# lyuchenyang/Macaw-LLM

Measured on NVIDIA H100. Metric: multimodal prefill tokens/sec (img+audio+text->LLaMA), higher is better.
Workload: dtype fp16

## Files before the change

### macaw-llm_b200/csrc/gemm_wgmma.cu

```cuda
#include "common.cuh"
#include "ptx.cuh"
#include "../../include/macaw_b200.h"
#include <stdlib.h>

namespace mm {

struct GemmKParams {
  int M, N, K, batch, batch2;
  int m_tiles, n_tiles, num_k;
  int b_shared, b2_shared;
  void* C;
  long long ldc, c_bs, c_bs2;
  int c_fp32;
  int act;
  float alpha;
  const bf16* bias;
  long long bias_bs;
  const float* row_scale;
  const bf16* residual;
  long long ldr, r_bs, r_bs2;
  int res_row_mod;
  const float* rope_cos;
  const float* rope_sin;
  int rope_T, rope_cols;
// ... 589 lines not shown
            phase ^= 1;
          }
        }
      }
    }
    return;
  }

  const int q = warp & 3;
  const float* srow = sC + (q * 32 + lane) * LDS;
  if (EWG && warp >= 8) {
    if constexpr (EWG) setmaxnreg_inc<168>();
    GemmWork wk;
    for (int it = 0; gemm_work(p, worker, n_workers, total_tiles, it, wk); ++it) {
      const TileCoord t = tile_coord(wk.tile, p, m_units);
      const float rs = epi_row_scale(p, t, t.m_blk * kBlockM + q * 32 + lane);
      mbar_wait(staging_full, it & 1);
      for (int half = 0; half < 2; ++half) gemm_epilogue<BN, EPI>(p, t, wk, srow, rs, q, lane, half, q + 4 * half, worker, n_workers);
      mbar_arrive(staging_empty);
    }
    return;
  }

  if constexpr (EWG) setmaxnreg_inc<152>();
  const int wg = warp >> 2;
  int stage = 0;
  uint32_t phase = 0;
  GemmWork wk;
  for (int it = 0; gemm_work(p, worker, n_workers, total_tiles, it, wk); ++it) {
    const TileCoord t = tile_coord(wk.tile, p, m_units);
    {
      float acc[BN / 2];
#pragma unroll
      for (int i = 0; i < BN / 2; ++i) acc[i] = 0.f;
      int prev = -1;
      for (int kb = wk.kb0; kb < wk.kb1; ++kb) {
        mbar_wait(&full_bar[stage], phase);
        const uint32_t a_addr = smem_u32(sA + stage * kABytes) + wg * 8192;
        const uint32_t b_addr = smem_u32(sB + stage * B_BYTES);
        const uint64_t a_desc = make_sdesc_sw128(a_addr, A_MN ? 8192 : 16, 1024);
        const uint64_t b_desc = make_sdesc_sw128(b_addr, B_MN ? 8192 : 16, 1024);
        wgmma_fence();
#pragma unroll
        for (int kk = 0; kk < kBlockK / 16; ++kk)
          wgmma_tile<BN, F16, A_MN ? 1 : 0, B_MN ? 1 : 0>(acc, a_desc + static_cast<uint64_t>(A_MN ? kk * 128 : kk * 2),
                                                         b_desc + static_cast<uint64_t>(B_MN ? kk * 128 : kk * 2));
        wgmma_commit();
        wgmma_wait<1>();
        if (prev >= 0) {
          __syncwarp();
          if (lane == 0) mbar_arrive(&empty_bar[prev]);
        }
        prev = stage;
        if (++stage == STAGES) {
          stage = 0;
          phase ^= 1;
        }
      }
      wgmma_wait<0>();
      fence_regs(acc);
      __syncwarp();
      if (lane == 0) mbar_arrive(&empty_bar[prev]);
      if constexpr (EWG) mbar_wait(staging_empty, (it & 1) ^ 1);
      else consumer_sync();
      const int r0 = wg * 64 + q * 16 + (lane >> 2);
      const int c0 = 2 * (lane & 3);
#pragma unroll
      for (int j = 0; j < BN / 8; ++j) {
        *reinterpret_cast<float2*>(sC + r0 * LDS + 8 * j + c0) = make_float2(acc[4 * j], acc[4 * j + 1]);
        *reinterpret_cast<float2*>(sC + (r0 + 8) * LDS + 8 * j + c0) = make_float2(acc[4 * j + 2], acc[4 * j + 3]);
      }
      if constexpr (EWG) {
        mbar_arrive(staging_full);
        continue;
      }
      consumer_sync();
    }
    const int half = warp >> 2;
    const float rs = wk.role == 1 ? 1.0f : epi_row_scale(p, t, t.m_blk * kBlockM + q * 32 + lane);
    gemm_epilogue<BN, EPI>(p, t, wk, srow, rs, q, lane, half, warp, worker, n_workers);
  }
}

typedef CUresult (*EncodeTiledFn)(CUtensorMap*, CUtensorMapDataType, cuuint32_t, void*, const cuuint64_t*,
                                  const cuuint64_t*, const cuuint32_t*, const cuuint32_t*, CUtensorMapInterleave,
                                  CUtensorMapSwizzle, CUtensorMapL2promotion, CUtensorMapFloatOOBfill);

static EncodeTiledFn get_encode_fn() {
  static EncodeTiledFn fn = nullptr;
  if (fn == nullptr) {
    void* p = nullptr;
    cudaDriverEntryPointQueryResult q;
    if (cudaGetDriverEntryPoint("cuTensorMapEncodeTiled", &p, cudaEnableDefault, &q) == cudaSuccess &&
        q == cudaDriverEntryPointSuccess)
      fn = reinterpret_cast<EncodeTiledFn>(p);
  }
  return fn;
}

int make_map(CUtensorMap* m, const void* ptr, uint64_t inner, uint64_t rows, uint64_t batch, uint64_t batch2,
             int64_t ld, int64_t bs, int64_t bs2, uint32_t box_rows) {
  EncodeTiledFn fn = get_encode_fn();
  if (fn == nullptr) {
    set_error("cuTensorMapEncodeTiled entry point unavailable (no CUDA driver?)");
    return 1;
  }
  cuuint64_t dims[4] = {inner, rows, batch, batch2};
  if (bs <= 0) bs = static_cast<int64_t>(rows) * ld;
  if (bs2 <= 0) bs2 = static_cast<int64_t>(batch) * bs;
  cuuint64_t strides[3] = {static_cast<cuuint64_t>(ld) * 2, static_cast<cuuint64_t>(bs) * 2,
                           static_cast<cuuint64_t>(bs2) * 2};
  cuuint32_t box[4] = {64, box_rows, 1, 1};
  cuuint32_t estr[4] = {1, 1, 1, 1};
  CUresult r = fn(m, CU_TENSOR_MAP_DATA_TYPE_BFLOAT16, 4, const_cast<void*>(ptr), dims, strides, box, estr,
                  CU_TENSOR_MAP_INTERLEAVE_NONE, CU_TENSOR_MAP_SWIZZLE_128B, CU_TENSOR_MAP_L2_PROMOTION_L2_256B,
                  CU_TENSOR_MAP_FLOAT_OOB_FILL_NONE);
  if (r != CUDA_SUCCESS) {
    set_error("cuTensorMapEncodeTiled failed (%d): ptr=%p dims={%llu,%llu,%llu,%llu} ld=%lld bs=%lld bs2=%lld box_rows=%u",
              static_cast<int>(r), ptr, (unsigned long long)inner, (unsigned long long)rows,
              (unsigned long long)batch, (unsigned long long)batch2, (long long)ld, (long long)bs, (long long)bs2,
              box_rows);
    return 1;
  }
  return 0;
}


static int& streamk_mode() {
  static int mode = []() { const char* e = getenv("MACAW_B200_GEMM_STREAMK"); const int v = e ? atoi(e) : 1; return v < 0 || v > 2 ? 1 : v; }();
  return mode;
}

static int& overlap_mode() {
  static int mode = []() { const char* e = getenv("MACAW_B200_GEMM_OVERLAP"); const int v = e ? atoi(e) : 1; return v < 0 || v > 1 ? 1 : v; }();
  return mode;
}

template <int BN, int EPI, bool B_MN, bool A_MN = false>
static int launch_gemm(const CUtensorMap& ta, const CUtensorMap& tb, const GemmKParams& p, bool f16, bool ewg,
                       cudaStream_t st) {
  if (ewg && p.sk_tiles != 0) {
    set_error("mm_gemm_fwd: the epilogue-warpgroup kernel takes no stream-K tail");
    return 1;
  }
  static bool attr_set[2][2][kMaxDevices] = {};
  constexpr size_t smem = gemm_smem_bytes(BN);
  auto kern = f16 ? (ewg ? gemm_bf16_kernel<BN, EPI, B_MN, A_MN, true, true> : gemm_bf16_kernel<BN, EPI, B_MN, A_MN, true, false>)
                  : (ewg ? gemm_bf16_kernel<BN, EPI, B_MN, A_MN, false, true> : gemm_bf16_kernel<BN, EPI, B_MN, A_MN, false, false>);
  if (int rc = ensure_smem_attr(kern, smem, attr_set[f16 ? 1 : 0][ewg ? 1 : 0], "mm_gemm_fwd")) return rc;
  const int total = p.batch * p.batch2 * p.m_tiles * p.n_tiles;
  const int grid = (total < num_sms() && p.sk_tiles == 0) ? total : num_sms();
  cudaError_t e = launch_kernel(kern, dim3(grid), dim3(ewg ? kGemmThreadsEwg : kGemmThreads), smem, st, 1, ta, tb, p);
  if (e != cudaSuccess) {
    set_error("mm_gemm_fwd: launch failed: %s", cudaGetErrorString(e));
    return 2;
  }
  return check_launch("mm_gemm_fwd");
}

}

using namespace mm;

static int32_t gemm_dispatch(const mm_gemm_args* a, void* stream, mm_gemm_schedule* plan) {
  MM_REQUIRE(a != nullptr, "mm_gemm_fwd: null args");
  MM_REQUIRE(a->M > 0 && a->N > 0 && a->K > 0 && a->batch > 0 && a->batch2 >= 0,
             "mm_gemm_fwd: bad shape M=%d N=%d K=%d batch=%d batch2=%d", a->M, a->N, a->K, a->batch, a->batch2);
  const int batch2 = a->batch2 > 0 ? a->batch2 : 1;
  MM_REQUIRE(a->A && a->B && a->C, "mm_gemm_fwd: null operand");
  MM_REQUIRE((reinterpret_cast<uintptr_t>(a->A) & 15) == 0 && (reinterpret_cast<uintptr_t>(a->B) & 15) == 0,
             "mm_gemm_fwd: A/B must be 16-byte aligned");
  MM_REQUIRE(a->lda % 8 == 0 && a->ldb % 8 == 0, "mm_gemm_fwd: lda/ldb must be multiples of 8 elements (lda=%lld ldb=%lld)",
             (long long)a->lda, (long long)a->ldb);
  MM_REQUIRE(a->batch == 1 || (a->a_bs % 8 == 0 && a->b_bs % 8 == 0), "mm_gemm_fwd: batch strides must be multiples of 8");
  MM_REQUIRE(batch2 == 1 || (a->a_bs2 % 8 == 0 && a->b_bs2 % 8 == 0), "mm_gemm_fwd: batch2 strides must be multiples of 8");
  MM_REQUIRE(a->epi >= MM_EPI_STD && a->epi <= MM_EPI_ROPE, "mm_gemm_fwd: bad epilogue %d", a->epi);

  GemmKParams p;
  p.M = a->M; p.N = a->N; p.K = a->K; p.batch = a->batch; p.batch2 = batch2;
  p.num_k = (a->K + kBlockK - 1) / kBlockK;
  p.m_tiles = (a->M + kBlockM - 1) / kBlockM;
  p.b_shared = (a->batch > 1 && a->b_bs == 0) ? 1 : 0;
  p.b2_shared = (batch2 > 1 && a->b_bs2 == 0) ? 1 : 0;
  p.C = a->C; p.ldc = a->ldc; p.c_bs = a->c_bs; p.c_bs2 = a->c_bs2; p.c_fp32 = a->c_fp32;
  p.act = a->act; p.alpha = a->alpha;
  p.bias = reinterpret_cast<const bf16*>(a->bias); p.bias_bs = a->bias_bs;
  p.row_scale = a->row_scale;
  p.residual = reinterpret_cast<const bf16*>(a->residual); p.ldr = a->ldr; p.r_bs = a->r_bs; p.r_bs2 = a->r_bs2;
  p.res_row_mod = a->res_row_mod;
  p.rope_cos = a->rope_cos; p.rope_sin = a->rope_sin; p.rope_T = a->rope_T; p.rope_cols = a->rope_cols;
  p.rope_pos = a->rope_pos;
  p.c_trans = a->c_trans;
  p.c_fp16 = a->c_fp16;
  p.aux_f16 = act_f16() ? 1 : 0;
  p.bias_rs = a->bias_rs; p.bias2 = reinterpret_cast<const bf16*>(a->bias2); p.bias2_rs = a->bias2_rs;
  p.sumsq_out = a->sumsq_out; p.sumsq_parts = (a->N + 31) / 32;
  p.rs_sumsq = a->rs_sumsq; p.rs_parts = a->rs_parts; p.rs_eps = a->rs_eps;
  MM_REQUIRE(a->sumsq_out == nullptr || (a->epi == MM_EPI_STD && !a->c_trans && !a->c_fp32 && a->batch == 1 && batch2 == 1 &&
                                         a->N % 32 == 0),
             "mm_gemm_fwd: sumsq_out needs the standard epilogue, 16-bit output, no batching and N %% 32 == 0");
  MM_REQUIRE(a->rs_sumsq == nullptr || (a->rs_parts > 0 && a->rs_parts % 4 == 0 && !a->c_trans && a->batch == 1 && batch2 == 1 &&
                                        (reinterpret_cast<uintptr_t>(a->rs_sumsq) & 15) == 0),
             "mm_gemm_fwd: rs_sumsq needs rs_parts %% 4 == 0, a 16-byte aligned buffer and no batching");
  MM_REQUIRE(!(a->c_fp16 && a->c_fp32), "mm_gemm_fwd: c_fp16 and c_fp32 are exclusive");
  MM_REQUIRE((a->a_fp16 != 0) == (a->b_fp16 != 0),
             "mm_gemm_fwd: A and B must share one 16-bit format (wgmma takes no mixed f16 x bf16 operands)");
  MM_REQUIRE((!a->bias_rs && !a->bias2 && !a->bias2_rs) || (a->epi == MM_EPI_STD && !a->c_trans),
             "mm_gemm_fwd: row-scaled bias terms need the standard, non-transposed epilogue");
  MM_REQUIRE(!(a->c_fp16 && a->c_fp32), "mm_gemm_fwd: c_fp16 and c_fp32 are exclusive");
  MM_REQUIRE(!a->c_trans || (a->epi == MM_EPI_STD && a->batch == 1 && batch2 == 1),
             "mm_gemm_fwd: c_trans needs the standard epilogue and no batching");

  const int esz = a->c_fp32 ? 4 : 2;
  bool vec = (reinterpret_cast<uintptr_t>(a->C) % 16 == 0) && ((a->ldc * esz) % 16 == 0) &&
             ((a->c_bs * esz) % 16 == 0) && ((a->c_bs2 * esz) % 16 == 0);
  if (a->bias) vec = vec && (reinterpret_cast<uintptr_t>(a->bias) % 16 == 0) && (a->bias_bs % 8 == 0);
  if (a->residual)
    vec = vec && (reinterpret_cast<uintptr_t>(a->residual) % 16 == 0) && (a->ldr % 8 == 0) && (a->r_bs % 8 == 0) &&
          (a->r_bs2 % 8 == 0);
  p.vec_ok = vec ? 1 : 0;

  const int sms = num_sms();
  int BN = kMaxBN;
  if (a->epi == MM_EPI_ROPE) {
    MM_REQUIRE(a->N % 128 == 0 && a->rope_cos && a->rope_sin && a->rope_T > 0 && vec && a->rope_cols % 128 == 0,
               "mm_gemm_fwd: RoPE epilogue needs N %% 128 == 0, cos/sin tables and vector-aligned C");
  } else if (a->epi == MM_EPI_SWIGLU) {
    MM_REQUIRE(a->N % 64 == 0, "mm_gemm_fwd: SwiGLU epilogue needs N %% 64 == 0");
  } else {
    const int cands[3] = {128, 64, 32};
    const long long kcost[3] = {512, 282, 192};
    long long best = -1;
    BN = 32;
    for (int i = 0; i < 3; ++i) {
      const int bn = cands[i];
      if (a->b_mn_major && bn < 64) continue;
      if (bn > 32 && a->N <= bn / 2) continue;
      const long long tiles = (long long)a->batch * batch2 * p.m_tiles * ((a->N + bn - 1) / bn);
      const long long waves = (tiles + sms - 1) / sms;
      const long long cost = waves * ((long long)p.num_k * kcost[i] + 2 * kcost[i]);
      if (best < 0 || cost < best) {
        best = cost;
        BN = bn;
      }
    }
    if (a->b_mn_major && BN < 64) BN = 64;
  }
  p.n_tiles = (a->N + BN - 1) / BN;
  static const int gm_env = []() { const char* e = getenv("MACAW_B200_GEMM_GROUPM"); return e ? atoi(e) : 0; }();
  const long long tiles = (long long)a->batch * batch2 * p.m_tiles * p.n_tiles;
  {
    const long long unit_bytes = (long long)kBlockM * a->K * 2;
    long long g = ((16LL << 20) + unit_bytes / 2) / unit_bytes;
    g = g < 2 ? 2 : (g > 32 ? 32 : g);
    p.group_m = gm_env > 0 ? gm_env : static_cast<int>(g);
  }
  p.sk_tiles = 0; p.sk_first = 0; p.sk_ws = nullptr; p.sk_flags = nullptr;
  const int sk_env = streamk_mode();
  if (sk_env != 0 && a->sk_workspace != nullptr && p.num_k >= 8 && tiles > sms &&
      static_cast<long long>(sms) * p.num_k * (sms + 1) < (1LL << 31)) {
    const int rem = static_cast<int>(tiles % sms);
    const long long need = 8192 + static_cast<long long>(sms) * kBlockM * BN * 4;
    const bool pays = sk_env == 2 || static_cast<long long>(sms - rem) * p.num_k * BN >= 3400LL * 256;
    if (rem > 0 && pays && a->sk_workspace_bytes >= need &&
        (reinterpret_cast<uintptr_t>(a->sk_workspace) & 15) == 0) {
      p.sk_tiles = rem;
      p.sk_first = static_cast<int>(tiles - rem);
      p.sk_flags = reinterpret_cast<int*>(a->sk_workspace);
      p.sk_ws = reinterpret_cast<float*>(reinterpret_cast<char*>(a->sk_workspace) + 8192);
    }
  }
  MM_REQUIRE(!a->a_mn_major || (a->b_mn_major && a->epi == MM_EPI_STD && !a->c_trans),
             "mm_gemm_fwd: MN-major A needs MN-major B and the standard epilogue");
  MM_REQUIRE(!a->b_mn_major || a->epi == MM_EPI_STD, "mm_gemm_fwd: MN-major B only with the standard epilogue");
  if (plan != nullptr) {
    plan->block_n = BN;
    plan->pairs = 0;
    plan->m_tiles = p.m_tiles;
    plan->n_tiles = p.n_tiles;
    plan->k_blocks = p.num_k;
    plan->units = tiles;
    plan->workers = sms;
    plan->grid = static_cast<int>((tiles < sms && p.sk_tiles == 0) ? tiles : sms);
    plan->waves = static_cast<int>((tiles + sms - 1) / sms);
    plan->group_m = p.group_m;
    plan->streamk_tiles = p.sk_tiles;
    plan->smem_bytes = static_cast<int32_t>(gemm_smem_bytes(BN));
    plan->vectorised_epilogue = p.vec_ok;
    return 0;
  }
  CUtensorMap ta, tb;
  if (a->a_mn_major) {
    if (make_map(&ta, a->A, a->M, a->K, a->batch, batch2, a->lda, a->a_bs, a->a_bs2, 64)) return 1;
  } else if (make_map(&ta, a->A, a->K, a->M, a->batch, batch2, a->lda, a->a_bs, a->a_bs2, kBlockM)) {
    return 1;
  }
  const uint64_t b_batch = p.b_shared ? 1 : a->batch;
  const uint64_t b_batch2 = p.b2_shared ? 1 : batch2;
  if (!a->b_mn_major) {
    if (make_map(&tb, a->B, a->K, a->N, b_batch, b_batch2, a->ldb, a->b_bs, a->b_bs2, BN)) return 1;
  } else {
    if (make_map(&tb, a->B, a->N, a->K, b_batch, b_batch2, a->ldb, a->b_bs, a->b_bs2, 64)) return 1;
  }
  cudaStream_t st = reinterpret_cast<cudaStream_t>(stream);
  const bool f16 = a->a_fp16 != 0;
  const bool ewg = overlap_mode() == 1 && p.num_k >= kEwgMinKBlocks && p.sk_tiles == 0;

#define MM_LAUNCH(BN_, EPI_, MN_) return launch_gemm<BN_, EPI_, MN_>(ta, tb, p, f16, ewg, st)
  if (a->epi == MM_EPI_ROPE) MM_LAUNCH(128, MM_EPI_ROPE, false);
  if (a->epi == MM_EPI_SWIGLU) MM_LAUNCH(128, MM_EPI_SWIGLU, false);
  if (a->a_mn_major) {
    if (BN == 128) return launch_gemm<128, MM_EPI_STD, true, true>(ta, tb, p, f16, ewg, st);
    return launch_gemm<64, MM_EPI_STD, true, true>(ta, tb, p, f16, ewg, st);
  }
  if (a->b_mn_major) {
    if (BN == 128) MM_LAUNCH(128, MM_EPI_STD, true);
    MM_LAUNCH(64, MM_EPI_STD, true);
  }
  if (BN == 128) MM_LAUNCH(128, MM_EPI_STD, false);
  if (BN == 64) MM_LAUNCH(64, MM_EPI_STD, false);
  MM_LAUNCH(32, MM_EPI_STD, false);
#undef MM_LAUNCH
}

extern "C" int32_t mm_gemm_fwd(const mm_gemm_args* a, void* stream) { return gemm_dispatch(a, stream, nullptr); }

extern "C" int32_t mm_gemm_plan(const mm_gemm_args* a, mm_gemm_schedule* plan) {
  MM_REQUIRE(plan != nullptr, "mm_gemm_plan: null plan");
  return gemm_dispatch(a, nullptr, plan);
}

extern "C" int32_t mm_gemm_streamk_mode(int32_t mode) {
  const int prev = streamk_mode();
  if (mode >= 0 && mode <= 2) streamk_mode() = mode;
  return prev;
}

extern "C" int32_t mm_gemm_overlap_mode(int32_t mode) {
  const int prev = overlap_mode();
  if (mode >= 0 && mode <= 1) overlap_mode() = mode;
  return prev;
}

extern "C" int64_t mm_gemm_streamk_workspace_bytes(void) {
  return 8192 + static_cast<int64_t>(num_sms()) * kBlockM * kMaxBN * 4;
}


namespace mm {
__global__ void splitk_reduce_kernel(const float* __restrict__ part, int splits, int M, int N,
                                     const bf16* __restrict__ bias, bf16* __restrict__ out, long long ldo, int out_fp16,
                                     int bias_f16) {
  const long long total = static_cast<long long>(M) * N;
  for (long long i = blockIdx.x * static_cast<long long>(blockDim.x) + threadIdx.x; i < total;
       i += static_cast<long long>(gridDim.x) * blockDim.x) {
    const int m = static_cast<int>(i / N), n = static_cast<int>(i % N);
    float acc = bias ? aux_ld(bias, n, bias_f16) : 0.0f;
    for (int s = 0; s < splits; ++s) acc += part[static_cast<long long>(s) * total + i];
    if (out_fp16)
      reinterpret_cast<__half*>(out)[static_cast<long long>(m) * ldo + n] = __float2half_rn(acc);
    else
      out[static_cast<long long>(m) * ldo + n] = __float2bfloat16(acc);
  }
}
}

extern "C" int32_t mm_splitk_reduce(const float* partial, int32_t splits, int32_t M, int32_t N, const void* bias,
                                    void* out, int64_t ldo, int32_t out_fp16, void* stream) {
  MM_REQUIRE(partial && out && splits > 0 && M > 0 && N > 0, "mm_splitk_reduce: bad arguments");
  const long long total = static_cast<long long>(M) * N;
  int blocks = static_cast<int>((total + 255) / 256);
  if (blocks > num_sms() * 8) blocks = num_sms() * 8;
  splitk_reduce_kernel<<<blocks, 256, 0, reinterpret_cast<cudaStream_t>(stream)>>>(
      partial, splits, M, N, reinterpret_cast<const bf16*>(bias), reinterpret_cast<bf16*>(out), ldo, out_fp16,
      act_f16() ? 1 : 0);
  return check_launch("mm_splitk_reduce");
}
```

### macaw-llm_b200/csrc/ptx.cuh

```cuda
#pragma once
#include <cuda_runtime.h>
#include <cuda_bf16.h>
#include <cuda_fp16.h>
#include <cuda.h>
#include <stdint.h>

namespace mm {

__device__ __forceinline__ uint32_t smem_u32(const void* p) {
  return static_cast<uint32_t>(__cvta_generic_to_shared(p));
}

__device__ __forceinline__ uint32_t lane_id() { return threadIdx.x & 31; }

__device__ __forceinline__ uint32_t elect_one() {
  uint32_t pred = 0;
  asm volatile(
      "{\n"
      ".reg .pred px;\n"
      "elect.sync _|px, 0xFFFFFFFF;\n"
      "selp.b32 %0, 1, 0, px;\n"
      "}\n"
      : "=r"(pred));
  return pred;
// ... 74 lines not shown
      : "memory");
}
constexpr uint64_t kEvictNormal = 0x1000000000000000ull;
constexpr uint64_t kEvictFirst = 0x12F0000000000000ull;
constexpr uint64_t kEvictLast = 0x14F0000000000000ull;

__device__ __forceinline__ uint64_t make_sdesc_sw128(uint32_t smem_addr, uint32_t lbo_bytes, uint32_t sbo_bytes) {
  uint64_t d = 0;
  d |= static_cast<uint64_t>((smem_addr & 0x3FFFF) >> 4);
  d |= static_cast<uint64_t>((lbo_bytes >> 4) & 0x3FFF) << 16;
  d |= static_cast<uint64_t>((sbo_bytes >> 4) & 0x3FFF) << 32;
  d |= static_cast<uint64_t>(1) << 62;
  return d;
}

__device__ __forceinline__ void wgmma_fence() { asm volatile("wgmma.fence.sync.aligned;" ::: "memory"); }
__device__ __forceinline__ void wgmma_commit() { asm volatile("wgmma.commit_group.sync.aligned;" ::: "memory"); }
template <int N>
__device__ __forceinline__ void wgmma_wait() {
  asm volatile("wgmma.wait_group.sync.aligned %0;" ::"n"(N) : "memory");
}
template <int N>
__device__ __forceinline__ void fence_regs(float (&d)[N]) {
#pragma unroll
  for (int i = 0; i < N; ++i) asm volatile("" : "+f"(d[i])::"memory");
}

__device__ __forceinline__ void stage_ld32(const float* s, uint32_t (&r)[32]) {
#pragma unroll
  for (int i = 0; i < 8; ++i) {
    const float4 f = reinterpret_cast<const float4*>(s)[i];
    r[4 * i] = __float_as_uint(f.x);
    r[4 * i + 1] = __float_as_uint(f.y);
    r[4 * i + 2] = __float_as_uint(f.z);
    r[4 * i + 3] = __float_as_uint(f.w);
  }
}

template <bool F16, int TA, int TB>
__device__ __forceinline__ void wgmma_ss_n32(float (&d)[16], uint64_t a, uint64_t b, uint32_t scale_d) {
  if constexpr (F16)
    asm volatile(
        "{\n.reg .pred p;\nsetp.ne.b32 p, %18, 0;\n"
        "wgmma.mma_async.sync.aligned.m64n32k16.f32.f16.f16 {%0, %1, %2, %3, %4, %5, %6, %7, %8, %9, %10, %11, %12, %13, %14, %15}, %16, %17, p, 1, 1, %19, %20;\n}\n"
        : "+f"(d[0]), "+f"(d[1]), "+f"(d[2]), "+f"(d[3]), "+f"(d[4]), "+f"(d[5]), "+f"(d[6]), "+f"(d[7]), "+f"(d[8]), "+f"(d[9]), "+f"(d[10]), "+f"(d[11]), "+f"(d[12]), "+f"(d[13]), "+f"(d[14]), "+f"(d[15])
        : "l"(a), "l"(b), "r"(scale_d), "n"(TA), "n"(TB));
  else
    asm volatile(
        "{\n.reg .pred p;\nsetp.ne.b32 p, %18, 0;\n"
        "wgmma.mma_async.sync.aligned.m64n32k16.f32.bf16.bf16 {%0, %1, %2, %3, %4, %5, %6, %7, %8, %9, %10, %11, %12, %13, %14, %15}, %16, %17, p, 1, 1, %19, %20;\n}\n"
        : "+f"(d[0]), "+f"(d[1]), "+f"(d[2]), "+f"(d[3]), "+f"(d[4]), "+f"(d[5]), "+f"(d[6]), "+f"(d[7]), "+f"(d[8]), "+f"(d[9]), "+f"(d[10]), "+f"(d[11]), "+f"(d[12]), "+f"(d[13]), "+f"(d[14]), "+f"(d[15])
        : "l"(a), "l"(b), "r"(scale_d), "n"(TA), "n"(TB));
}
template <bool F16, int TA, int TB>
__device__ __forceinline__ void wgmma_ss_n64(float (&d)[32], uint64_t a, uint64_t b, uint32_t scale_d) {
  if constexpr (F16)
    asm volatile(
        "{\n.reg .pred p;\nsetp.ne.b32 p, %34, 0;\n"
        "wgmma.mma_async.sync.aligned.m64n64k16.f32.f16.f16 {%0, %1, %2, %3, %4, %5, %6, %7, %8, %9, %10, %11, %12, %13, %14, %15, %16, %17, %18, %19, %20, %21, %22, %23, %24, %25, %26, %27, %28, %29, %30, %31}, %32, %33, p, 1, 1, %35, %36;\n}\n"
        : "+f"(d[0]), "+f"(d[1]), "+f"(d[2]), "+f"(d[3]), "+f"(d[4]), "+f"(d[5]), "+f"(d[6]), "+f"(d[7]), "+f"(d[8]), "+f"(d[9]), "+f"(d[10]), "+f"(d[11]), "+f"(d[12]), "+f"(d[13]), "+f"(d[14]), "+f"(d[15]), "+f"(d[16]), "+f"(d[17]), "+f"(d[18]), "+f"(d[19]), "+f"(d[20]), "+f"(d[21]), "+f"(d[22]), "+f"(d[23]), "+f"(d[24]), "+f"(d[25]), "+f"(d[26]), "+f"(d[27]), "+f"(d[28]), "+f"(d[29]), "+f"(d[30]), "+f"(d[31])
        : "l"(a), "l"(b), "r"(scale_d), "n"(TA), "n"(TB));
  else
    asm volatile(
        "{\n.reg .pred p;\nsetp.ne.b32 p, %34, 0;\n"
        "wgmma.mma_async.sync.aligned.m64n64k16.f32.bf16.bf16 {%0, %1, %2, %3, %4, %5, %6, %7, %8, %9, %10, %11, %12, %13, %14, %15, %16, %17, %18, %19, %20, %21, %22, %23, %24, %25, %26, %27, %28, %29, %30, %31}, %32, %33, p, 1, 1, %35, %36;\n}\n"
        : "+f"(d[0]), "+f"(d[1]), "+f"(d[2]), "+f"(d[3]), "+f"(d[4]), "+f"(d[5]), "+f"(d[6]), "+f"(d[7]), "+f"(d[8]), "+f"(d[9]), "+f"(d[10]), "+f"(d[11]), "+f"(d[12]), "+f"(d[13]), "+f"(d[14]), "+f"(d[15]), "+f"(d[16]), "+f"(d[17]), "+f"(d[18]), "+f"(d[19]), "+f"(d[20]), "+f"(d[21]), "+f"(d[22]), "+f"(d[23]), "+f"(d[24]), "+f"(d[25]), "+f"(d[26]), "+f"(d[27]), "+f"(d[28]), "+f"(d[29]), "+f"(d[30]), "+f"(d[31])
        : "l"(a), "l"(b), "r"(scale_d), "n"(TA), "n"(TB));
}
template <bool F16, int TA, int TB>
__device__ __forceinline__ void wgmma_ss_n128(float (&d)[64], uint64_t a, uint64_t b, uint32_t scale_d) {
  if constexpr (F16)
    asm volatile(
        "{\n.reg .pred p;\nsetp.ne.b32 p, %66, 0;\n"
        "wgmma.mma_async.sync.aligned.m64n128k16.f32.f16.f16 {%0, %1, %2, %3, %4, %5, %6, %7, %8, %9, %10, %11, %12, %13, %14, %15, %16, %17, %18, %19, %20, %21, %22, %23, %24, %25, %26, %27, %28, %29, %30, %31, %32, %33, %34, %35, %36, %37, %38, %39, %40, %41, %42, %43, %44, %45, %46, %47, %48, %49, %50, %51, %52, %53, %54, %55, %56, %57, %58, %59, %60, %61, %62, %63}, %64, %65, p, 1, 1, %67, %68;\n}\n"
        : "+f"(d[0]), "+f"(d[1]), "+f"(d[2]), "+f"(d[3]), "+f"(d[4]), "+f"(d[5]), "+f"(d[6]), "+f"(d[7]), "+f"(d[8]), "+f"(d[9]), "+f"(d[10]), "+f"(d[11]), "+f"(d[12]), "+f"(d[13]), "+f"(d[14]), "+f"(d[15]), "+f"(d[16]), "+f"(d[17]), "+f"(d[18]), "+f"(d[19]), "+f"(d[20]), "+f"(d[21]), "+f"(d[22]), "+f"(d[23]), "+f"(d[24]), "+f"(d[25]), "+f"(d[26]), "+f"(d[27]), "+f"(d[28]), "+f"(d[29]), "+f"(d[30]), "+f"(d[31]), "+f"(d[32]), "+f"(d[33]), "+f"(d[34]), "+f"(d[35]), "+f"(d[36]), "+f"(d[37]), "+f"(d[38]), "+f"(d[39]), "+f"(d[40]), "+f"(d[41]), "+f"(d[42]), "+f"(d[43]), "+f"(d[44]), "+f"(d[45]), "+f"(d[46]), "+f"(d[47]), "+f"(d[48]), "+f"(d[49]), "+f"(d[50]), "+f"(d[51]), "+f"(d[52]), "+f"(d[53]), "+f"(d[54]), "+f"(d[55]), "+f"(d[56]), "+f"(d[57]), "+f"(d[58]), "+f"(d[59]), "+f"(d[60]), "+f"(d[61]), "+f"(d[62]), "+f"(d[63])
        : "l"(a), "l"(b), "r"(scale_d), "n"(TA), "n"(TB));
  else
    asm volatile(
        "{\n.reg .pred p;\nsetp.ne.b32 p, %66, 0;\n"
        "wgmma.mma_async.sync.aligned.m64n128k16.f32.bf16.bf16 {%0, %1, %2, %3, %4, %5, %6, %7, %8, %9, %10, %11, %12, %13, %14, %15, %16, %17, %18, %19, %20, %21, %22, %23, %24, %25, %26, %27, %28, %29, %30, %31, %32, %33, %34, %35, %36, %37, %38, %39, %40, %41, %42, %43, %44, %45, %46, %47, %48, %49, %50, %51, %52, %53, %54, %55, %56, %57, %58, %59, %60, %61, %62, %63}, %64, %65, p, 1, 1, %67, %68;\n}\n"
        : "+f"(d[0]), "+f"(d[1]), "+f"(d[2]), "+f"(d[3]), "+f"(d[4]), "+f"(d[5]), "+f"(d[6]), "+f"(d[7]), "+f"(d[8]), "+f"(d[9]), "+f"(d[10]), "+f"(d[11]), "+f"(d[12]), "+f"(d[13]), "+f"(d[14]), "+f"(d[15]), "+f"(d[16]), "+f"(d[17]), "+f"(d[18]), "+f"(d[19]), "+f"(d[20]), "+f"(d[21]), "+f"(d[22]), "+f"(d[23]), "+f"(d[24]), "+f"(d[25]), "+f"(d[26]), "+f"(d[27]), "+f"(d[28]), "+f"(d[29]), "+f"(d[30]), "+f"(d[31]), "+f"(d[32]), "+f"(d[33]), "+f"(d[34]), "+f"(d[35]), "+f"(d[36]), "+f"(d[37]), "+f"(d[38]), "+f"(d[39]), "+f"(d[40]), "+f"(d[41]), "+f"(d[42]), "+f"(d[43]), "+f"(d[44]), "+f"(d[45]), "+f"(d[46]), "+f"(d[47]), "+f"(d[48]), "+f"(d[49]), "+f"(d[50]), "+f"(d[51]), "+f"(d[52]), "+f"(d[53]), "+f"(d[54]), "+f"(d[55]), "+f"(d[56]), "+f"(d[57]), "+f"(d[58]), "+f"(d[59]), "+f"(d[60]), "+f"(d[61]), "+f"(d[62]), "+f"(d[63])
        : "l"(a), "l"(b), "r"(scale_d), "n"(TA), "n"(TB));
}
template <bool F16, int TB>
__device__ __forceinline__ void wgmma_rs_n64(float (&d)[32], const uint32_t (&a)[4], uint64_t b, uint32_t scale_d) {
  if constexpr (F16)
    asm volatile(
        "{\n.reg .pred p;\nsetp.ne.b32 p, %37, 0;\n"
        "wgmma.mma_async.sync.aligned.m64n64k16.f32.f16.f16 {%0, %1, %2, %3, %4, %5, %6, %7, %8, %9, %10, %11, %12, %13, %14, %15, %16, %17, %18, %19, %20, %21, %22, %23, %24, %25, %26, %27, %28, %29, %30, %31}, {%32, %33, %34, %35}, %36, p, 1, 1, %38;\n}\n"
        : "+f"(d[0]), "+f"(d[1]), "+f"(d[2]), "+f"(d[3]), "+f"(d[4]), "+f"(d[5]), "+f"(d[6]), "+f"(d[7]), "+f"(d[8]), "+f"(d[9]), "+f"(d[10]), "+f"(d[11]), "+f"(d[12]), "+f"(d[13]), "+f"(d[14]), "+f"(d[15]), "+f"(d[16]), "+f"(d[17]), "+f"(d[18]), "+f"(d[19]), "+f"(d[20]), "+f"(d[21]), "+f"(d[22]), "+f"(d[23]), "+f"(d[24]), "+f"(d[25]), "+f"(d[26]), "+f"(d[27]), "+f"(d[28]), "+f"(d[29]), "+f"(d[30]), "+f"(d[31])
        : "r"(a[0]), "r"(a[1]), "r"(a[2]), "r"(a[3]), "l"(b), "r"(scale_d), "n"(TB));
  else
    asm volatile(
        "{\n.reg .pred p;\nsetp.ne.b32 p, %37, 0;\n"
        "wgmma.mma_async.sync.aligned.m64n64k16.f32.bf16.bf16 {%0, %1, %2, %3, %4, %5, %6, %7, %8, %9, %10, %11, %12, %13, %14, %15, %16, %17, %18, %19, %20, %21, %22, %23, %24, %25, %26, %27, %28, %29, %30, %31}, {%32, %33, %34, %35}, %36, p, 1, 1, %38;\n}\n"
        : "+f"(d[0]), "+f"(d[1]), "+f"(d[2]), "+f"(d[3]), "+f"(d[4]), "+f"(d[5]), "+f"(d[6]), "+f"(d[7]), "+f"(d[8]), "+f"(d[9]), "+f"(d[10]), "+f"(d[11]), "+f"(d[12]), "+f"(d[13]), "+f"(d[14]), "+f"(d[15]), "+f"(d[16]), "+f"(d[17]), "+f"(d[18]), "+f"(d[19]), "+f"(d[20]), "+f"(d[21]), "+f"(d[22]), "+f"(d[23]), "+f"(d[24]), "+f"(d[25]), "+f"(d[26]), "+f"(d[27]), "+f"(d[28]), "+f"(d[29]), "+f"(d[30]), "+f"(d[31])
        : "r"(a[0]), "r"(a[1]), "r"(a[2]), "r"(a[3]), "l"(b), "r"(scale_d), "n"(TB));
}
template <bool F16, int TB>
__device__ __forceinline__ void wgmma_rs_n128(float (&d)[64], const uint32_t (&a)[4], uint64_t b, uint32_t scale_d) {
  if constexpr (F16)
    asm volatile(
        "{\n.reg .pred p;\nsetp.ne.b32 p, %69, 0;\n"
        "wgmma.mma_async.sync.aligned.m64n128k16.f32.f16.f16 {%0, %1, %2, %3, %4, %5, %6, %7, %8, %9, %10, %11, %12, %13, %14, %15, %16, %17, %18, %19, %20, %21, %22, %23, %24, %25, %26, %27, %28, %29, %30, %31, %32, %33, %34, %35, %36, %37, %38, %39, %40, %41, %42, %43, %44, %45, %46, %47, %48, %49, %50, %51, %52, %53, %54, %55, %56, %57, %58, %59, %60, %61, %62, %63}, {%64, %65, %66, %67}, %68, p, 1, 1, %70;\n}\n"
        : "+f"(d[0]), "+f"(d[1]), "+f"(d[2]), "+f"(d[3]), "+f"(d[4]), "+f"(d[5]), "+f"(d[6]), "+f"(d[7]), "+f"(d[8]), "+f"(d[9]), "+f"(d[10]), "+f"(d[11]), "+f"(d[12]), "+f"(d[13]), "+f"(d[14]), "+f"(d[15]), "+f"(d[16]), "+f"(d[17]), "+f"(d[18]), "+f"(d[19]), "+f"(d[20]), "+f"(d[21]), "+f"(d[22]), "+f"(d[23]), "+f"(d[24]), "+f"(d[25]), "+f"(d[26]), "+f"(d[27]), "+f"(d[28]), "+f"(d[29]), "+f"(d[30]), "+f"(d[31]), "+f"(d[32]), "+f"(d[33]), "+f"(d[34]), "+f"(d[35]), "+f"(d[36]), "+f"(d[37]), "+f"(d[38]), "+f"(d[39]), "+f"(d[40]), "+f"(d[41]), "+f"(d[42]), "+f"(d[43]), "+f"(d[44]), "+f"(d[45]), "+f"(d[46]), "+f"(d[47]), "+f"(d[48]), "+f"(d[49]), "+f"(d[50]), "+f"(d[51]), "+f"(d[52]), "+f"(d[53]), "+f"(d[54]), "+f"(d[55]), "+f"(d[56]), "+f"(d[57]), "+f"(d[58]), "+f"(d[59]), "+f"(d[60]), "+f"(d[61]), "+f"(d[62]), "+f"(d[63])
        : "r"(a[0]), "r"(a[1]), "r"(a[2]), "r"(a[3]), "l"(b), "r"(scale_d), "n"(TB));
  else
    asm volatile(
        "{\n.reg .pred p;\nsetp.ne.b32 p, %69, 0;\n"
        "wgmma.mma_async.sync.aligned.m64n128k16.f32.bf16.bf16 {%0, %1, %2, %3, %4, %5, %6, %7, %8, %9, %10, %11, %12, %13, %14, %15, %16, %17, %18, %19, %20, %21, %22, %23, %24, %25, %26, %27, %28, %29, %30, %31, %32, %33, %34, %35, %36, %37, %38, %39, %40, %41, %42, %43, %44, %45, %46, %47, %48, %49, %50, %51, %52, %53, %54, %55, %56, %57, %58, %59, %60, %61, %62, %63}, {%64, %65, %66, %67}, %68, p, 1, 1, %70;\n}\n"
        : "+f"(d[0]), "+f"(d[1]), "+f"(d[2]), "+f"(d[3]), "+f"(d[4]), "+f"(d[5]), "+f"(d[6]), "+f"(d[7]), "+f"(d[8]), "+f"(d[9]), "+f"(d[10]), "+f"(d[11]), "+f"(d[12]), "+f"(d[13]), "+f"(d[14]), "+f"(d[15]), "+f"(d[16]), "+f"(d[17]), "+f"(d[18]), "+f"(d[19]), "+f"(d[20]), "+f"(d[21]), "+f"(d[22]), "+f"(d[23]), "+f"(d[24]), "+f"(d[25]), "+f"(d[26]), "+f"(d[27]), "+f"(d[28]), "+f"(d[29]), "+f"(d[30]), "+f"(d[31]), "+f"(d[32]), "+f"(d[33]), "+f"(d[34]), "+f"(d[35]), "+f"(d[36]), "+f"(d[37]), "+f"(d[38]), "+f"(d[39]), "+f"(d[40]), "+f"(d[41]), "+f"(d[42]), "+f"(d[43]), "+f"(d[44]), "+f"(d[45]), "+f"(d[46]), "+f"(d[47]), "+f"(d[48]), "+f"(d[49]), "+f"(d[50]), "+f"(d[51]), "+f"(d[52]), "+f"(d[53]), "+f"(d[54]), "+f"(d[55]), "+f"(d[56]), "+f"(d[57]), "+f"(d[58]), "+f"(d[59]), "+f"(d[60]), "+f"(d[61]), "+f"(d[62]), "+f"(d[63])
        : "r"(a[0]), "r"(a[1]), "r"(a[2]), "r"(a[3]), "l"(b), "r"(scale_d), "n"(TB));
}

__device__ __forceinline__ uint32_t pack_bf16x2(float lo, float hi) {
  __nv_bfloat162 v = __floats2bfloat162_rn(lo, hi);
  return *reinterpret_cast<uint32_t*>(&v);
}
__device__ __forceinline__ uint32_t pack_f16x2(float lo, float hi) {
  __half2 v = __floats2half2_rn(lo, hi);
  return *reinterpret_cast<uint32_t*>(&v);
}
__device__ __forceinline__ float bf16lo(uint32_t v) { return __uint_as_float(v << 16); }
__device__ __forceinline__ float bf16hi(uint32_t v) { return __uint_as_float(v & 0xFFFF0000u); }

template <bool F16>
__device__ __forceinline__ float cvt_in(uint16_t raw) {
  if constexpr (F16) return __half2float(__ushort_as_half(raw));
  return __uint_as_float(static_cast<uint32_t>(raw) << 16);
}
template <bool F16>
__device__ __forceinline__ uint16_t cvt_out(float v) {
  if constexpr (F16) return __half_as_ushort(__float2half_rn(v));
  return __bfloat16_as_ushort(__float2bfloat16(v));
}
template <bool F16>
__device__ __forceinline__ uint32_t pack2(float lo, float hi) {
  if constexpr (F16) return pack_f16x2(lo, hi);
  return pack_bf16x2(lo, hi);
}
template <bool F16>
__device__ __forceinline__ void unpack2(uint32_t v, float& lo, float& hi) {
  if constexpr (F16) {
    const float2 f = __half22float2(*reinterpret_cast<const __half2*>(&v));
    lo = f.x;
    hi = f.y;
  } else {
    lo = bf16lo(v);
    hi = bf16hi(v);
  }
}
template <bool F16>
__device__ __forceinline__ void unpack8t(const uint4& u, float (&f)[8]) {
  unpack2<F16>(u.x, f[0], f[1]);
  unpack2<F16>(u.y, f[2], f[3]);
  unpack2<F16>(u.z, f[4], f[5]);
  unpack2<F16>(u.w, f[6], f[7]);
}
template <bool F16>
__device__ __forceinline__ uint4 pack8t(const float (&f)[8]) {
  return make_uint4(pack2<F16>(f[0], f[1]), pack2<F16>(f[2], f[3]), pack2<F16>(f[4], f[5]), pack2<F16>(f[6], f[7]));
}
template <bool F16>
__device__ __forceinline__ float ldv(__nv_bfloat16 v) { return cvt_in<F16>(__bfloat16_as_ushort(v)); }
template <bool F16>
__device__ __forceinline__ __nv_bfloat16 stv(float v) { return __ushort_as_bfloat16(cvt_out<F16>(v)); }
// ... 3 lines not shown
```

Measured before the change: 33500.

## Add wide 128x256 wgmma GEMM kernel with dedicated epilogue warpgroup

Adds a persistent GEMM kernel in which each CTA computes a pair of adjacent N tiles (BN=256) using m64n256k16 wgmma, with two consumer warpgroups and a third warpgroup handling the epilogue through a staged shared-memory tile. Loading the wider B tile per A tile raises operand reuse and halves the A traffic per output. The default overlap mode becomes 2, which routes large non-batched, K-major GEMMs with an even number of N tiles to this kernel. The trade-offs are fewer pipeline stages (3), higher register pressure handled via setmaxnreg, and a serialized two-sided epilogue handoff.

```diff
diff --git a/macaw-llm_b200/csrc/gemm_wgmma.cu b/macaw-llm_b200/csrc/gemm_wgmma.cu
--- a/macaw-llm_b200/csrc/gemm_wgmma.cu
+++ b/macaw-llm_b200/csrc/gemm_wgmma.cu
@@ -695,6 +695,164 @@
   }
 }
 
+constexpr int kWideThreads = 384;
+constexpr int kWideStages = 3;
+constexpr uint32_t kWideBBytes = 2 * kMaxBN * kBlockK * 2;
+constexpr size_t kWideSmemBytes =
+    1024 + kWideStages * (kABytes + kWideBBytes) + (size_t)kBlockM * gemm_stage_ld(kMaxBN) * 4 + 256;
+static_assert(kWideSmemBytes <= 227 * 1024, "wide GEMM: ring + staging tile exceed an sm_90 block's shared memory");
+constexpr int kWideRegsConsumer = 184, kWideRegsEpilogue = 136;
+static_assert(2 * kWideRegsConsumer + kWideRegsEpilogue <= 3 * 168, "wide GEMM: register budget");
+
+__device__ __forceinline__ TileCoord pair_coord(int idx, const GemmKParams& p) {
+  const int n_pairs = p.n_tiles / 2;
+  const int in_group = p.group_m * n_pairs;
+  const int g = idx / in_group;
+  const int first_m = g * p.group_m;
+  const int gsz = min(p.m_tiles - first_m, p.group_m);
+  const int rr = idx - g * in_group;
+  TileCoord t;
+  t.b = t.b_lo = t.b_hi = 0;
+  t.m_blk = first_m + rr % gsz;
+  t.n_blk = 2 * (rr / gsz);
+  return t;
+}
+
+template <int EPI, bool F16>
+__global__ void __launch_bounds__(kWideThreads, 1)
+gemm_wide_kernel(const __grid_constant__ CUtensorMap tmA, const __grid_constant__ CUtensorMap tmB, const GemmKParams p) {
+  constexpr int BN = kMaxBN;
+  constexpr int LDS = gemm_stage_ld(BN);
+  extern __shared__ uint8_t smem_raw[];
+  uint8_t* smem = reinterpret_cast<uint8_t*>((reinterpret_cast<uintptr_t>(smem_raw) + 1023) & ~uintptr_t(1023));
+  uint8_t* sA = smem;
+  uint8_t* sB = smem + kWideStages * kABytes;
+  float* sC = reinterpret_cast<float*>(sB + kWideStages * kWideBBytes);
+  uint64_t* full_bar = reinterpret_cast<uint64_t*>(sC + kBlockM * LDS);
+  uint64_t* empty_bar = full_bar + kWideStages;
+  uint64_t* staging_full = empty_bar + kWideStages;
+  uint64_t* staging_empty = staging_full + 1;
+
+  const int warp = threadIdx.x >> 5;
+  const int lane = threadIdx.x & 31;
+  const int worker = static_cast<int>(blockIdx.x);
+  const int n_workers = static_cast<int>(gridDim.x);
+  const int total_pairs = p.m_tiles * (p.n_tiles / 2);
+
+  if (warp == 0 && elect_one()) {
+    tma_prefetch_desc(&tmA);
+    tma_prefetch_desc(&tmB);
+    for (int s = 0; s < kWideStages; ++s) {
+      mbar_init(&full_bar[s], 1);
+      mbar_init(&empty_bar[s], 8);
+    }
+    mbar_init(staging_full, 256);
+    mbar_init(staging_empty, 128);
+    fence_mbar_init();
+  }
+  __syncthreads();
+  griddep_launch();
+  griddep_wait();
+
+  const int q = warp & 3;
+  if (warp >= 8) {
+    setmaxnreg_dec<kWideRegsEpilogue>();
+    const float* srow = sC + (q * 32 + lane) * LDS;
+    GemmWork wk;
+    wk.tile = 0; wk.kb0 = 0; wk.kb1 = p.num_k; wk.role = 0; wk.c0 = 0; wk.nc = 0;
+    for (int u = worker; u < total_pairs; u += n_workers) {
+      TileCoord t = pair_coord(u, p);
+      const float rs = epi_row_scale(p, t, t.m_blk * kBlockM + q * 32 + lane);
+#pragma unroll 1
+      for (int side = 0; side < 2; ++side) {
+        mbar_wait(staging_full, side);
+        for (int half = 0; half < 2; ++half)
+          gemm_epilogue<BN, EPI>(p, t, wk, srow, rs, q, lane, half, q + 4 * half, worker, n_workers);
+        mbar_arrive(staging_empty);
+        ++t.n_blk;
+      }
+    }
+    return;
+  }
+
+  setmaxnreg_inc<kWideRegsConsumer>();
+  const int wg = warp >> 2;
+  int stage = 0;
+  uint32_t phase = 0;
+  const bool loader = threadIdx.x == 0;
+  int ld_u = worker, ld_kb = 0, ld_stage = 0;
+  uint32_t ld_phase = 0;
+  TileCoord ld_t = pair_coord(worker, p);
+  auto load_next = [&]() {
+    if (ld_u >= total_pairs) return;
+    mbar_wait(&empty_bar[ld_stage], ld_phase ^ 1);
+    mbar_arrive_expect_tx(&full_bar[ld_stage], kABytes + kWideBBytes);
+    tma_load_4d(&tmA, &full_bar[ld_stage], sA + ld_stage * kABytes, ld_kb * kBlockK, ld_t.m_blk * kBlockM, 0, 0);
+    uint8_t* b = sB + ld_stage * kWideBBytes;
+    tma_load_4d(&tmB, &full_bar[ld_stage], b, ld_kb * kBlockK, ld_t.n_blk * BN, 0, 0);
+    tma_load_4d(&tmB, &full_bar[ld_stage], b + kWideBBytes / 2, ld_kb * kBlockK, (ld_t.n_blk + 1) * BN, 0, 0);
+    if (++ld_stage == kWideStages) {
+      ld_stage = 0;
+      ld_phase ^= 1;
+    }
+    if (++ld_kb == p.num_k) {
+      ld_kb = 0;
+      ld_u += n_workers;
+      if (ld_u < total_pairs) ld_t = pair_coord(ld_u, p);
+    }
+  };
+  if (loader)
+    for (int s = 0; s < kWideStages; ++s) load_next();
+  __syncwarp();
+  for (int u = worker; u < total_pairs; u += n_workers) {
+    float acc[2 * BN / 2];
+#pragma unroll
+    for (int i = 0; i < BN; ++i) acc[i] = 0.f;
+    int prev = -1;
+    for (int kb = 0; kb < p.num_k; ++kb) {
+      mbar_wait(&full_bar[stage], phase);
+      const uint64_t a_desc = make_sdesc_sw128(smem_u32(sA + stage * kABytes) + wg * 8192, 16, 1024);
+      const uint64_t b_desc = make_sdesc_sw128(smem_u32(sB + stage * kWideBBytes), 16, 1024);
+      wgmma_fence();
+#pragma unroll
+      for (int kk = 0; kk < kBlockK / 16; ++kk)
+        wgmma_ss_n256<F16, 0, 0>(acc, a_desc + static_cast<uint64_t>(kk * 2), b_desc + static_cast<uint64_t>(kk * 2), 1u);
+      wgmma_commit();
+      wgmma_wait<1>();
+      if (prev >= 0) {
+        __syncwarp();
+        if (lane == 0) mbar_arrive(&empty_bar[prev]);
+        if (loader) load_next();
+        __syncwarp();
+      }
+      prev = stage;
+      if (++stage == kWideStages) {
+        stage = 0;
+        phase ^= 1;
+      }
+    }
+    wgmma_wait<0>();
+    fence_regs(acc);
+    __syncwarp();
+    if (lane == 0) mbar_arrive(&empty_bar[prev]);
+    if (loader) load_next();
+    __syncwarp();
+    const int r0 = wg * 64 + q * 16 + (lane >> 2);
+    const int c0 = 2 * (lane & 3);
+#pragma unroll
+    for (int side = 0; side < 2; ++side) {
+      mbar_wait(staging_empty, side ^ 1);
+#pragma unroll
+      for (int j = 0; j < BN / 8; ++j) {
+        const int i = side * (BN / 2) + 4 * j;
+        *reinterpret_cast<float2*>(sC + r0 * LDS + 8 * j + c0) = make_float2(acc[i], acc[i + 1]);
+        *reinterpret_cast<float2*>(sC + (r0 + 8) * LDS + 8 * j + c0) = make_float2(acc[i + 2], acc[i + 3]);
+      }
+      mbar_arrive(staging_full);
+    }
+  }
+}
+
 typedef CUresult (*EncodeTiledFn)(CUtensorMap*, CUtensorMapDataType, cuuint32_t, void*, const cuuint64_t*,
                                   const cuuint64_t*, const cuuint32_t*, const cuuint32_t*, CUtensorMapInterleave,
                                   CUtensorMapSwizzle, CUtensorMapL2promotion, CUtensorMapFloatOOBfill);
@@ -745,7 +903,7 @@
 }
 
 static int& overlap_mode() {
-  static int mode = []() { const char* e = getenv("MACAW_B200_GEMM_OVERLAP"); const int v = e ? atoi(e) : 1; return v < 0 || v > 1 ? 1 : v; }();
+  static int mode = []() { const char* e = getenv("MACAW_B200_GEMM_OVERLAP"); const int v = e ? atoi(e) : 2; return v < 0 || v > 2 ? 2 : v; }();
   return mode;
 }
 
@@ -764,6 +922,21 @@
   const int total = p.batch * p.batch2 * p.m_tiles * p.n_tiles;
   const int grid = (total < num_sms() && p.sk_tiles == 0) ? total : num_sms();
   cudaError_t e = launch_kernel(kern, dim3(grid), dim3(ewg ? kGemmThreadsEwg : kGemmThreads), smem, st, 1, ta, tb, p);
+  if (e != cudaSuccess) {
+    set_error("mm_gemm_fwd: launch failed: %s", cudaGetErrorString(e));
+    return 2;
+  }
+  return check_launch("mm_gemm_fwd");
+}
+
+template <int EPI>
+static int launch_gemm_wide(const CUtensorMap& ta, const CUtensorMap& tb, const GemmKParams& p, bool f16, cudaStream_t st) {
+  static bool attr_set[2][kMaxDevices] = {};
+  auto kern = f16 ? gemm_wide_kernel<EPI, true> : gemm_wide_kernel<EPI, false>;
+  if (int rc = ensure_smem_attr(kern, kWideSmemBytes, attr_set[f16 ? 1 : 0], "mm_gemm_fwd")) return rc;
+  const int pairs = p.m_tiles * (p.n_tiles / 2);
+  cudaError_t e = launch_kernel(kern, dim3(pairs < num_sms() ? pairs : num_sms()), dim3(kWideThreads), kWideSmemBytes,
+                                st, 1, ta, tb, p);
   if (e != cudaSuccess) {
     set_error("mm_gemm_fwd: launch failed: %s", cudaGetErrorString(e));
     return 2;
@@ -917,7 +1090,13 @@
   }
   cudaStream_t st = reinterpret_cast<cudaStream_t>(stream);
   const bool f16 = a->a_fp16 != 0;
-  const bool ewg = overlap_mode() == 1 && p.num_k >= kEwgMinKBlocks && p.sk_tiles == 0;
+  const bool ewg = overlap_mode() >= 1 && p.num_k >= kEwgMinKBlocks && p.sk_tiles == 0;
+  if (overlap_mode() == 2 && ewg && BN == kMaxBN && !a->a_mn_major && !a->b_mn_major && !a->c_trans && a->batch == 1 &&
+      batch2 == 1 && p.n_tiles % 2 == 0 && tiles / 2 >= sms) {
+    if (a->epi == MM_EPI_ROPE) return launch_gemm_wide<MM_EPI_ROPE>(ta, tb, p, f16, st);
+    if (a->epi == MM_EPI_SWIGLU) return launch_gemm_wide<MM_EPI_SWIGLU>(ta, tb, p, f16, st);
+    return launch_gemm_wide<MM_EPI_STD>(ta, tb, p, f16, st);
+  }
 
 #define MM_LAUNCH(BN_, EPI_, MN_) return launch_gemm<BN_, EPI_, MN_>(ta, tb, p, f16, ewg, st)
   if (a->epi == MM_EPI_ROPE) MM_LAUNCH(128, MM_EPI_ROPE, false);
@@ -951,7 +1130,7 @@
 
 extern "C" int32_t mm_gemm_overlap_mode(int32_t mode) {
   const int prev = overlap_mode();
-  if (mode >= 0 && mode <= 1) overlap_mode() = mode;
+  if (mode >= 0 && mode <= 2) overlap_mode() = mode;
   return prev;
 }
 
diff --git a/macaw-llm_b200/csrc/ptx.cuh b/macaw-llm_b200/csrc/ptx.cuh
--- a/macaw-llm_b200/csrc/ptx.cuh
+++ b/macaw-llm_b200/csrc/ptx.cuh
@@ -180,6 +180,21 @@
         : "+f"(d[0]), "+f"(d[1]), "+f"(d[2]), "+f"(d[3]), "+f"(d[4]), "+f"(d[5]), "+f"(d[6]), "+f"(d[7]), "+f"(d[8]), "+f"(d[9]), "+f"(d[10]), "+f"(d[11]), "+f"(d[12]), "+f"(d[13]), "+f"(d[14]), "+f"(d[15]), "+f"(d[16]), "+f"(d[17]), "+f"(d[18]), "+f"(d[19]), "+f"(d[20]), "+f"(d[21]), "+f"(d[22]), "+f"(d[23]), "+f"(d[24]), "+f"(d[25]), "+f"(d[26]), "+f"(d[27]), "+f"(d[28]), "+f"(d[29]), "+f"(d[30]), "+f"(d[31]), "+f"(d[32]), "+f"(d[33]), "+f"(d[34]), "+f"(d[35]), "+f"(d[36]), "+f"(d[37]), "+f"(d[38]), "+f"(d[39]), "+f"(d[40]), "+f"(d[41]), "+f"(d[42]), "+f"(d[43]), "+f"(d[44]), "+f"(d[45]), "+f"(d[46]), "+f"(d[47]), "+f"(d[48]), "+f"(d[49]), "+f"(d[50]), "+f"(d[51]), "+f"(d[52]), "+f"(d[53]), "+f"(d[54]), "+f"(d[55]), "+f"(d[56]), "+f"(d[57]), "+f"(d[58]), "+f"(d[59]), "+f"(d[60]), "+f"(d[61]), "+f"(d[62]), "+f"(d[63])
         : "l"(a), "l"(b), "r"(scale_d), "n"(TA), "n"(TB));
 }
+template <bool F16, int TA, int TB>
+__device__ __forceinline__ void wgmma_ss_n256(float (&d)[128], uint64_t a, uint64_t b, uint32_t scale_d) {
+  if constexpr (F16)
+    asm volatile(
+        "{\n.reg .pred p;\nsetp.ne.b32 p, %130, 0;\n"
+        "wgmma.mma_async.sync.aligned.m64n256k16.f32.f16.f16 {%0, %1, %2, %3, %4, %5, %6, %7, %8, %9, %10, %11, %12, %13, %14, %15, %16, %17, %18, %19, %20, %21, %22, %23, %24, %25, %26, %27, %28, %29, %30, %31, %32, %33, %34, %35, %36, %37, %38, %39, %40, %41, %42, %43, %44, %45, %46, %47, %48, %49, %50, %51, %52, %53, %54, %55, %56, %57, %58, %59, %60, %61, %62, %63, %64, %65, %66, %67, %68, %69, %70, %71, %72, %73, %74, %75, %76, %77, %78, %79, %80, %81, %82, %83, %84, %85, %86, %87, %88, %89, %90, %91, %92, %93, %94, %95, %96, %97, %98, %99, %100, %101, %102, %103, %104, %105, %106, %107, %108, %109, %110, %111, %112, %113, %114, %115, %116, %117, %118, %119, %120, %121, %122, %123, %124, %125, %126, %127}, %128, %129, p, 1, 1, %131, %132;\n}\n"
+        : "+f"(d[0]), "+f"(d[1]), "+f"(d[2]), "+f"(d[3]), "+f"(d[4]), "+f"(d[5]), "+f"(d[6]), "+f"(d[7]), "+f"(d[8]), "+f"(d[9]), "+f"(d[10]), "+f"(d[11]), "+f"(d[12]), "+f"(d[13]), "+f"(d[14]), "+f"(d[15]), "+f"(d[16]), "+f"(d[17]), "+f"(d[18]), "+f"(d[19]), "+f"(d[20]), "+f"(d[21]), "+f"(d[22]), "+f"(d[23]), "+f"(d[24]), "+f"(d[25]), "+f"(d[26]), "+f"(d[27]), "+f"(d[28]), "+f"(d[29]), "+f"(d[30]), "+f"(d[31]), "+f"(d[32]), "+f"(d[33]), "+f"(d[34]), "+f"(d[35]), "+f"(d[36]), "+f"(d[37]), "+f"(d[38]), "+f"(d[39]), "+f"(d[40]), "+f"(d[41]), "+f"(d[42]), "+f"(d[43]), "+f"(d[44]), "+f"(d[45]), "+f"(d[46]), "+f"(d[47]), "+f"(d[48]), "+f"(d[49]), "+f"(d[50]), "+f"(d[51]), "+f"(d[52]), "+f"(d[53]), "+f"(d[54]), "+f"(d[55]), "+f"(d[56]), "+f"(d[57]), "+f"(d[58]), "+f"(d[59]), "+f"(d[60]), "+f"(d[61]), "+f"(d[62]), "+f"(d[63]), "+f"(d[64]), "+f"(d[65]), "+f"(d[66]), "+f"(d[67]), "+f"(d[68]), "+f"(d[69]), "+f"(d[70]), "+f"(d[71]), "+f"(d[72]), "+f"(d[73]), "+f"(d[74]), "+f"(d[75]), "+f"(d[76]), "+f"(d[77]), "+f"(d[78]), "+f"(d[79]), "+f"(d[80]), "+f"(d[81]), "+f"(d[82]), "+f"(d[83]), "+f"(d[84]), "+f"(d[85]), "+f"(d[86]), "+f"(d[87]), "+f"(d[88]), "+f"(d[89]), "+f"(d[90]), "+f"(d[91]), "+f"(d[92]), "+f"(d[93]), "+f"(d[94]), "+f"(d[95]), "+f"(d[96]), "+f"(d[97]), "+f"(d[98]), "+f"(d[99]), "+f"(d[100]), "+f"(d[101]), "+f"(d[102]), "+f"(d[103]), "+f"(d[104]), "+f"(d[105]), "+f"(d[106]), "+f"(d[107]), "+f"(d[108]), "+f"(d[109]), "+f"(d[110]), "+f"(d[111]), "+f"(d[112]), "+f"(d[113]), "+f"(d[114]), "+f"(d[115]), "+f"(d[116]), "+f"(d[117]), "+f"(d[118]), "+f"(d[119]), "+f"(d[120]), "+f"(d[121]), "+f"(d[122]), "+f"(d[123]), "+f"(d[124]), "+f"(d[125]), "+f"(d[126]), "+f"(d[127])
+        : "l"(a), "l"(b), "r"(scale_d), "n"(TA), "n"(TB));
+  else
+    asm volatile(
+        "{\n.reg .pred p;\nsetp.ne.b32 p, %130, 0;\n"
+        "wgmma.mma_async.sync.aligned.m64n256k16.f32.bf16.bf16 {%0, %1, %2, %3, %4, %5, %6, %7, %8, %9, %10, %11, %12, %13, %14, %15, %16, %17, %18, %19, %20, %21, %22, %23, %24, %25, %26, %27, %28, %29, %30, %31, %32, %33, %34, %35, %36, %37, %38, %39, %40, %41, %42, %43, %44, %45, %46, %47, %48, %49, %50, %51, %52, %53, %54, %55, %56, %57, %58, %59, %60, %61, %62, %63, %64, %65, %66, %67, %68, %69, %70, %71, %72, %73, %74, %75, %76, %77, %78, %79, %80, %81, %82, %83, %84, %85, %86, %87, %88, %89, %90, %91, %92, %93, %94, %95, %96, %97, %98, %99, %100, %101, %102, %103, %104, %105, %106, %107, %108, %109, %110, %111, %112, %113, %114, %115, %116, %117, %118, %119, %120, %121, %122, %123, %124, %125, %126, %127}, %128, %129, p, 1, 1, %131, %132;\n}\n"
+        : "+f"(d[0]), "+f"(d[1]), "+f"(d[2]), "+f"(d[3]), "+f"(d[4]), "+f"(d[5]), "+f"(d[6]), "+f"(d[7]), "+f"(d[8]), "+f"(d[9]), "+f"(d[10]), "+f"(d[11]), "+f"(d[12]), "+f"(d[13]), "+f"(d[14]), "+f"(d[15]), "+f"(d[16]), "+f"(d[17]), "+f"(d[18]), "+f"(d[19]), "+f"(d[20]), "+f"(d[21]), "+f"(d[22]), "+f"(d[23]), "+f"(d[24]), "+f"(d[25]), "+f"(d[26]), "+f"(d[27]), "+f"(d[28]), "+f"(d[29]), "+f"(d[30]), "+f"(d[31]), "+f"(d[32]), "+f"(d[33]), "+f"(d[34]), "+f"(d[35]), "+f"(d[36]), "+f"(d[37]), "+f"(d[38]), "+f"(d[39]), "+f"(d[40]), "+f"(d[41]), "+f"(d[42]), "+f"(d[43]), "+f"(d[44]), "+f"(d[45]), "+f"(d[46]), "+f"(d[47]), "+f"(d[48]), "+f"(d[49]), "+f"(d[50]), "+f"(d[51]), "+f"(d[52]), "+f"(d[53]), "+f"(d[54]), "+f"(d[55]), "+f"(d[56]), "+f"(d[57]), "+f"(d[58]), "+f"(d[59]), "+f"(d[60]), "+f"(d[61]), "+f"(d[62]), "+f"(d[63]), "+f"(d[64]), "+f"(d[65]), "+f"(d[66]), "+f"(d[67]), "+f"(d[68]), "+f"(d[69]), "+f"(d[70]), "+f"(d[71]), "+f"(d[72]), "+f"(d[73]), "+f"(d[74]), "+f"(d[75]), "+f"(d[76]), "+f"(d[77]), "+f"(d[78]), "+f"(d[79]), "+f"(d[80]), "+f"(d[81]), "+f"(d[82]), "+f"(d[83]), "+f"(d[84]), "+f"(d[85]), "+f"(d[86]), "+f"(d[87]), "+f"(d[88]), "+f"(d[89]), "+f"(d[90]), "+f"(d[91]), "+f"(d[92]), "+f"(d[93]), "+f"(d[94]), "+f"(d[95]), "+f"(d[96]), "+f"(d[97]), "+f"(d[98]), "+f"(d[99]), "+f"(d[100]), "+f"(d[101]), "+f"(d[102]), "+f"(d[103]), "+f"(d[104]), "+f"(d[105]), "+f"(d[106]), "+f"(d[107]), "+f"(d[108]), "+f"(d[109]), "+f"(d[110]), "+f"(d[111]), "+f"(d[112]), "+f"(d[113]), "+f"(d[114]), "+f"(d[115]), "+f"(d[116]), "+f"(d[117]), "+f"(d[118]), "+f"(d[119]), "+f"(d[120]), "+f"(d[121]), "+f"(d[122]), "+f"(d[123]), "+f"(d[124]), "+f"(d[125]), "+f"(d[126]), "+f"(d[127])
+        : "l"(a), "l"(b), "r"(scale_d), "n"(TA), "n"(TB));
+}
 template <bool F16, int TB>
 __device__ __forceinline__ void wgmma_rs_n64(float (&d)[32], const uint32_t (&a)[4], uint64_t b, uint32_t scale_d) {
   if constexpr (F16)
```

New measurement: 38580 (median of 6 runs). 1.15x the previous value.
